# kotaro-kinoshita/yomitoku

Hardware: NVIDIA H100
Metric: pages/sec (DBNet->PARSeq OCR, synthetic 1600x1200 pages, ~200 crops/page) (higher is better)
Workload: dtype f16

## Files before the change

yomitoku_b200/csrc/gemm_tc.cu:

```cuda
#include "gemm_tc.h"

#include <cstdarg>
#include <cstdlib>
#include <cstdio>
#include <cstring>
#include <atomic>
#include <mutex>
#include <vector>

#include "ptx.cuh"

namespace ytk {

static thread_local char g_err[512] = "";
void set_error(const char* fmt, ...) {
    va_list ap;
    va_start(ap, fmt);
    vsnprintf(g_err, sizeof(g_err), fmt, ap);
    va_end(ap);
}
const char* last_error() { return g_err; }

static std::atomic<long long> g_launches{0};
void count_launch(int n) { g_launches.fetch_add(n, std::memory_order_relaxed); }
// ... 22 lines not shown
        int dev = 0;
        cudaGetDevice(&dev);
        cudaDeviceGetAttribute(&n, cudaDevAttrMultiProcessorCount, dev);
        if (n <= 0) n = 132;
    }
    return n;
}

constexpr int kBlockM = 128;
constexpr int kBlockK = 64;
constexpr int kABytes = kBlockM * kBlockK * 2;
constexpr int kThreads = 384;
constexpr int kProducerWarp = 8;
constexpr int kStagePitch = 80;
constexpr int kEpiStageBytes = 8 * 32 * kStagePitch;
constexpr int kAccPitch = 68;
constexpr int kAccBytes = 2 * 64 * kAccPitch * 4;

constexpr int kEpiBufBytes = 32 * 64;
constexpr int epi_tma_nbuf(int ) { return 2; }
constexpr int kSmemLimit = 232448;
constexpr int kSmemFixed = 1024  + 1024  + 512 ;

template <int BLOCK_N, int EPI_BYTES = kEpiStageBytes>
struct TileCfg {
    static constexpr int kBBytes = BLOCK_N * kBlockK * 2;
    static constexpr int kStageBytes = kABytes + kBBytes;
    static constexpr int kRingBudget = kSmemLimit - kSmemFixed - kAccBytes - EPI_BYTES;
    static constexpr int kStages = (kRingBudget / kStageBytes) > 8 ? 8 : (kRingBudget / kStageBytes);
    static constexpr int kRingBytes = kStages * kStageBytes;
    static constexpr int kSmemBytes = kRingBytes + kAccBytes + EPI_BYTES + kSmemFixed;
    static_assert(kStages >= 3, "K pipeline depth");
// ... 36 lines not shown
    int t2 = m_tile / a.tiles_w;
    int th = t2 % a.tiles_h;
    t.img = t2 / a.tiles_h;
    t.h0 = th * (kBlockM >> a.bw_log2);
    t.w0 = tw << a.bw_log2;
    t.n0 = n_tile * block_n;
    return t;
}

template <int BLOCK_N, int RESID, int DIRECT>
using KernelCfg = TileCfg<BLOCK_N, DIRECT == 2 ? 8 * epi_tma_nbuf(RESID) * kEpiBufBytes : kEpiStageBytes>;

template <int BLOCK_N, int OUT_F32, int RESID, int MODE, int DIRECT>
__global__ void __launch_bounds__(kThreads, 1) gemm_tc_kernel(const __grid_constant__ GemmMaps maps,
                                                              const __grid_constant__ GemmArgs args) {
    using Cfg = KernelCfg<BLOCK_N, RESID, DIRECT>;
    constexpr int kEpiBytes = Cfg::kSmemBytes - Cfg::kRingBytes - kAccBytes - kSmemFixed;
    constexpr int stage_bytes = Cfg::kStageBytes;
    constexpr int nstages = Cfg::kStages;
    extern __shared__ uint8_t smem_raw[];
    const uint32_t raw_addr = smem_u32(smem_raw);
    uint8_t* smem = smem_raw + ((1024u - (raw_addr & 1023u)) & 1023u);
    const int worker = static_cast<int>(blockIdx.x);
    const int n_workers = static_cast<int>(gridDim.x);

    float* acc_smem = reinterpret_cast<float*>(smem + Cfg::kRingBytes);
    uint8_t* epi_stage = smem + Cfg::kRingBytes + kAccBytes;
    float* fin_w = reinterpret_cast<float*>(epi_stage + kEpiBytes);
    uint64_t* full_bar = reinterpret_cast<uint64_t*>(epi_stage + kEpiBytes + 1024);
    uint64_t* empty_bar = full_bar + 8;
    [[maybe_unused]] uint64_t* rbar_base = empty_bar + 8;

    const int warp = threadIdx.x >> 5;
    const int lane = threadIdx.x & 31;

    if (threadIdx.x == 0) {
        for (int i = 0; i < nstages; ++i) {
            mbar_init(&full_bar[i], 1);
            mbar_init(&empty_bar[i], 8);
        }
        if constexpr (DIRECT == 2 && RESID != 0) {
            for (int i = 0; i < 32; ++i) mbar_init(&rbar_base[i], 1);
        }
        fence_mbar_init();
        tma_prefetch_desc(&maps.a[0]);
        tma_prefetch_desc(&maps.b);
        if constexpr (DIRECT == 2) {
            tma_prefetch_desc(&maps.out);
            if constexpr (RESID != 0) {
                tma_prefetch_desc(&maps.resid);
                tma_prefetch_desc(&maps.resid_pf);
            }
        }
    }
// ... 38 lines not shown
                    tma_load_4d(sb, &maps.b, &full_bar[stage], kb * kBlockK, tc.n0, 0, 0);
                    if (++cb == args.kpt) {
                        cb = 0;
                        ++tap;
                    }
                    if (++stage == nstages) {
                        stage = 0;
                        phase ^= 1u;
                    }
                }
            }
        }
    } else {
        setmaxnreg_inc<232>();
        const int wg = warp >> 2, wl = warp & 3;
        const int q = 2 * wg + (wl & 1);
        const int wset = wl >> 1;
        float* acc_buf = acc_smem + wg * 64 * kAccPitch;
        const float* my_acc = acc_buf + ((wl & 1) * 32 + lane) * kAccPitch;
        float acc[BLOCK_N / 2];
#pragma unroll
        for (int i = 0; i < BLOCK_N / 2; ++i) acc[i] = 0.f;
        int ring_stage = 0;
        uint32_t ring_phase = 0;
        auto mma_tile = [&]() {
            const uint32_t a_off = static_cast<uint32_t>(wg * 64 * 128);
            int prev = -1;
            for (int kb = 0; kb < num_kb; ++kb) {
                mbar_wait(&full_bar[ring_stage], ring_phase);
                const uint32_t a_addr = smem_u32(smem + ring_stage * stage_bytes);
                const uint64_t da = wgmma_desc_sw128(a_addr + a_off);
                const uint64_t db = wgmma_desc_sw128(a_addr + kABytes);
                reg_fence(acc);
                wgmma_fence();
#pragma unroll
                for (int k = 0; k < kBlockK / 16; ++k)
                    wgmma_ss<BLOCK_N>(acc, da + static_cast<uint64_t>(2 * k), db + static_cast<uint64_t>(2 * k),
                                      (kb | k) != 0 ? 1u : 0u);
                wgmma_commit();
                wgmma_wait<1>();
                reg_fence(acc);
                if (prev >= 0) {
                    __syncwarp();
                    if (lane == 0) mbar_arrive(&empty_bar[prev]);
                }
                prev = ring_stage;
                if (++ring_stage == nstages) {
                    ring_stage = 0;
                    ring_phase ^= 1u;
                }
            }
            wgmma_wait<0>();
            reg_fence(acc);
            __syncwarp();
            if (lane == 0) mbar_arrive(&empty_bar[prev]);
        };
        auto dump_slice = [&](int s) {
            named_bar_sync(1 + wg, 128);
            const int r0 = wl * 16 + (lane >> 2), c2 = (lane & 3) * 2;
#pragma unroll
            for (int j = 0; j < BLOCK_N / 8; ++j) {
                if ((j >> 3) == s) {
                    float* p = acc_buf + r0 * kAccPitch + (j & 7) * 8 + c2;
                    *reinterpret_cast<float2*>(p) = make_float2(acc[4 * j], acc[4 * j + 1]);
                    *reinterpret_cast<float2*>(p + 8 * kAccPitch) = make_float2(acc[4 * j + 2], acc[4 * j + 3]);
                }
            }
            named_bar_sync(1 + wg, 128);
        };
        auto load_chunk = [&](int c, float (&f)[32]) {
            const float4* a4 = reinterpret_cast<const float4*>(my_acc + (c & 1) * 32);
#pragma unroll
            for (int j = 0; j < 8; ++j) {
                const float4 x = a4[j];
                f[4 * j + 0] = x.x;
                f[4 * j + 1] = x.y;
                f[4 * j + 2] = x.z;
                f[4 * j + 3] = x.w;
            }
        };
        if constexpr (DIRECT == 2) {
            static_assert(MODE == EPI_NORMAL, "TMA epilogue: plain stores only");
            static_assert(RESID == 0 || (RESID == 2) == (OUT_F32 != 0), "TMA epilogue: residual and output boxes match");
            constexpr int NBUF = epi_tma_nbuf(RESID);
            constexpr int LOOK = NBUF - 1;
            constexpr int CPP = OUT_F32 ? 16 : 32;
            constexpr int NPASS = 32 / CPP;
            const int bw_mask = (1 << args.bw_log2) - 1;
            const int qw = (q * 32) & bw_mask;
            const int qh = (q * 32) >> args.bw_log2;
            uint8_t* bufs = epi_stage + warp * (NBUF * kEpiBufBytes);
            [[maybe_unused]] uint64_t* rbar = rbar_base + warp * 4;
            const int sw = args.epi_swz ? ((lane >> 1) & 3) : 0;
            const int row_off = lane * 64;
            [[maybe_unused]] int pf_u = worker, pf_c = wset, pf_p = 0, pf_g = 0;
            [[maybe_unused]] TileCoord pf_tc{};
            [[maybe_unused]] auto pf_seek = [&]() {
                while (pf_u < total_units) {
                    pf_tc = decode_tile(args, pf_u, BLOCK_N);
                    if (pf_c < BLOCK_N / 32 && pf_tc.n0 + pf_c * 32 + pf_p * CPP < args.Cout) return;
                    pf_c = wset;
                    pf_p = 0;
                    pf_u += n_workers;
                }
            };
            [[maybe_unused]] auto pf_step = [&]() {
                if (++pf_p == NPASS) {
                    pf_p = 0;
                    pf_c += 2;
                }
                pf_seek();
            };
            [[maybe_unused]] auto pf_issue = [&]() {
                const int b = pf_g % NBUF;
                mbar_expect_tx(&rbar[b], kEpiBufBytes);
                tma_load_4d(bufs + b * kEpiBufBytes, &maps.resid, &rbar[b], pf_tc.n0 + pf_c * 32 + pf_p * CPP,
                            pf_tc.w0 + qw, pf_tc.h0 + qh, pf_tc.img);
                ++pf_g;
            };
            if constexpr (RESID != 0) {
                if (lane == 0) {
                    pf_seek();
                    for (int k = 0; k < LOOK && pf_u < total_units; ++k) {
                        pf_issue();
                        pf_step();
                    }
                }
            }
            int gc = 0;
            for (int u = worker; u < total_units; u += n_workers) {
                const TileCoord tc = decode_tile(args, u, BLOCK_N);
                mma_tile();
#pragma unroll 1
                for (int c = 0; c < BLOCK_N / 32; ++c) {
                    const int col0 = tc.n0 + c * 32;
                    if ((c & 1) == 0) {
                        if (col0 >= args.Cout) break;
                        dump_slice(c >> 1);
                    }
                    if ((c & 1) != wset || col0 >= args.Cout) continue;
                    float f[32];
                    load_chunk(c, f);
                    if (args.bias != nullptr) {
                        if (col0 + 32 <= args.Cout) {
                            const float4* b4 = reinterpret_cast<const float4*>(args.bias + col0);
#pragma unroll
                            for (int j = 0; j < 8; ++j) {
                                const float4 b = __ldg(b4 + j);
                                f[4 * j + 0] += b.x;
                                f[4 * j + 1] += b.y;
                                f[4 * j + 2] += b.z;
                                f[4 * j + 3] += b.w;
                            }
                        } else {
#pragma unroll
                            for (int j = 0; j < 32; ++j) f[j] += __ldg(args.bias + min(col0 + j, args.Cout - 1));
                        }
                    }
#pragma unroll
                    for (int p = 0; p < NPASS; ++p) {
                        if (col0 + p * CPP < args.Cout) {
                            const int b = gc % NBUF;
                            uint8_t* box = bufs + b * kEpiBufBytes;
                            uint8_t* my_row = box + row_off;
                            if constexpr (RESID != 0) {
                                mbar_wait(&rbar[b], static_cast<uint32_t>(gc / NBUF) & 1u);
#pragma unroll
                                for (int j = 0; j < 4; ++j) {
                                    const uint4 r = *reinterpret_cast<const uint4*>(my_row + ((j ^ sw) << 4));
                                    if constexpr (RESID == 2) {
                                        f[p * 16 + 4 * j + 0] += __uint_as_float(r.x);
                                        f[p * 16 + 4 * j + 1] += __uint_as_float(r.y);
                                        f[p * 16 + 4 * j + 2] += __uint_as_float(r.z);
                                        f[p * 16 + 4 * j + 3] += __uint_as_float(r.w);
                                    } else {
                                        const int e = p * CPP + 8 * j;
                                        f[e + 0] += op_lo(r.x); f[e + 1] += op_hi(r.x);
                                        f[e + 2] += op_lo(r.y); f[e + 3] += op_hi(r.y);
                                        f[e + 4] += op_lo(r.z); f[e + 5] += op_hi(r.z);
                                        f[e + 6] += op_lo(r.w); f[e + 7] += op_hi(r.w);
                                    }
                                }
                            } else {
                                if (lane == 0) bulk_wait_read<NBUF - 1>();
// ... 17 lines not shown
#pragma unroll
                            for (int j = 0; j < 4; ++j) {
                                uint4 o;
                                if constexpr (OUT_F32) {
                                    o.x = __float_as_uint(f[p * 16 + 4 * j + 0]);
                                    o.y = __float_as_uint(f[p * 16 + 4 * j + 1]);
                                    o.z = __float_as_uint(f[p * 16 + 4 * j + 2]);
                                    o.w = __float_as_uint(f[p * 16 + 4 * j + 3]);
                                } else {
                                    const int e = p * CPP + 8 * j;
                                    o.x = pack_op(f[e + 0], f[e + 1]);
                                    o.y = pack_op(f[e + 2], f[e + 3]);
                                    o.z = pack_op(f[e + 4], f[e + 5]);
                                    o.w = pack_op(f[e + 6], f[e + 7]);
                                }
                                *reinterpret_cast<uint4*>(my_row + ((j ^ sw) << 4)) = o;
                            }
                            fence_proxy_async_smem();
                            __syncwarp();
                            if (lane == 0) {
                                tma_store_4d(&maps.out, box, col0 + p * CPP, tc.w0 + qw, tc.h0 + qh, tc.img);
                                bulk_commit();
                                if constexpr (RESID != 0) {
                                    if (pf_u < total_units) {
                                        bulk_wait_read<1>();
                                        pf_issue();
                                        pf_step();
                                    }
                                }
                            }
                            ++gc;
                        }
                    }
                }
            }
            if (lane == 0) bulk_wait_read<0>();
            __syncwarp();
        } else {
        constexpr bool kFin = (MODE == EPI_CONVT_FINAL);
        constexpr bool kWide = (OUT_F32 != 0) || (RESID == 2);
        constexpr int CPP = kWide ? 16 : 32;
        constexpr int NPASS = 32 / CPP;
        constexpr int OESZ = OUT_F32 ? 4 : 2;
        constexpr int RESZ = (RESID == 2) ? 4 : 2;
        const int row = q * 32 + lane;
        const int bw_mask = (1 << args.bw_log2) - 1;
        uint8_t* stage = epi_stage + warp * (32 * kStagePitch);
        uint8_t* my_row = stage + lane * kStagePitch;
        const int piece = lane & 3;
        for (int u = worker; u < total_units; u += n_workers) {
            const TileCoord tc = decode_tile(args, u, BLOCK_N);
            const int hh = tc.h0 + (row >> args.bw_log2);
            const int ww = tc.w0 + (row & bw_mask);
            const bool row_ok = (hh < args.Ho) && (ww < args.Wo);
            int c_h[4], c_w[4];
            bool c_ok[4];
#pragma unroll
            for (int it = 0; it < 4; ++it) {
                const int rr = q * 32 + it * 8 + (lane >> 2);
                c_h[it] = tc.h0 + (rr >> args.bw_log2);
                c_w[it] = tc.w0 + (rr & bw_mask);
                c_ok[it] = (c_h[it] < args.Ho) && (c_w[it] < args.Wo);
            }
            mma_tile();
            [[maybe_unused]] float dots[4] = {0.f, 0.f, 0.f, 0.f};
            [[maybe_unused]] float rm_m = -INFINITY, rm_s = 0.f;
            [[maybe_unused]] int rm_i = 0x7fffffff;
#pragma unroll 1
            for (int c = 0; c < BLOCK_N / 32; ++c) {
                const int col0 = tc.n0 + c * 32;
                if ((c & 1) == 0) {
                    if (col0 >= args.Cout) break;
                    dump_slice(c >> 1);
                }
                if (((kFin ? (c >> 1) : c) & 1) != wset) continue;
                if (col0 >= args.Cout) continue;
                [[maybe_unused]] uint4 dres[RESID == 2 ? 8 : 4];
                if constexpr (RESID != 0 && !kFin && DIRECT == 1) {
                    const long long pixo = (static_cast<long long>(tc.img) * args.Ho + hh) * args.Wo + ww;
                    const bool fullc = row_ok && (col0 + 32 <= args.Cout);
                    const uint4* gp = reinterpret_cast<const uint4*>(reinterpret_cast<const char*>(args.resid) +
                                                                     (pixo * args.ldr + col0) * RESZ);
#pragma unroll
                    for (int j = 0; j < (RESID == 2 ? 8 : 4); ++j) dres[j] = fullc ? gp[j] : make_uint4(0, 0, 0, 0);
                }
                [[maybe_unused]] uint4 rres[NPASS][4];
                if constexpr (RESID != 0 && !kFin && DIRECT == 0) {
                    constexpr int per16r = 16 / RESZ;
                    int ocol_r = col0, sub_r = 0;
                    if constexpr (MODE == EPI_SHUFFLE2X) {
                        const int cq = args.Cout >> 2;
                        sub_r = col0 / cq;
                        ocol_r = col0 - sub_r * cq;
                    }
#pragma unroll
                    for (int p = 0; p < NPASS; ++p) {
                        const int validr = min(CPP, args.Cout - (col0 + p * CPP));
                        const int e0 = piece * per16r;
#pragma unroll
                        for (int it = 0; it < 4; ++it) {
                            rres[p][it] = make_uint4(0, 0, 0, 0);
                            if (c_ok[it] && e0 + per16r <= validr) {
                                const long long pixr =
                                    (static_cast<long long>(tc.img) * args.Ho + c_h[it]) * args.Wo + c_w[it];
                                const char* gp = reinterpret_cast<const char*>(args.resid) +
                                                 (pixr * args.ldr + ocol_r + p * CPP + e0) * RESZ;
                                rres[p][it] = *reinterpret_cast<const uint4*>(gp);
                            }
                        }
                    }
                }
                float f[32];
                load_chunk(c, f);
                if (args.bias != nullptr) {
                    if (col0 + 32 <= args.Cout) {
                        const float4* b4 = reinterpret_cast<const float4*>(args.bias + col0);
#pragma unroll
                        for (int j = 0; j < 8; ++j) {
                            const float4 b = __ldg(b4 + j);
                            f[4 * j + 0] += b.x;
                            f[4 * j + 1] += b.y;
                            f[4 * j + 2] += b.z;
                            f[4 * j + 3] += b.w;
                        }
                    } else {
#pragma unroll
                        for (int j = 0; j < 32; ++j) f[j] += __ldg(args.bias + min(col0 + j, args.Cout - 1));
                    }
// ... 17 lines not shown
                        for (int j = 0; j < 32; ++j) cs += __expf(f[j] - cm);
                    }
                    if (cm > rm_m) {
                        rm_s = rm_s * __expf(rm_m - cm) + cs;
                        rm_m = cm;
                        rm_i = ci;
                    } else {
                        rm_s += cs * __expf(cm - rm_m);
                    }
                } else if constexpr (kFin) {
                    const int chan0 = (c & 1) * 32;
#pragma unroll
                    for (int j = 0; j < 32; ++j) {
                        const float x = fmaxf(f[j], 0.f);
#pragma unroll
                        for (int k = 0; k < 4; ++k) dots[k] += x * fin_w[k * 64 + chan0 + j];
                    }
                    if (c & 1) {
                        if (row_ok) {
                            const int sub = c >> 1;
                            const long long oy = 2LL * (2 * hh + (sub >> 1)), ox = 2LL * (2 * ww + (sub & 1));
                            float* op = reinterpret_cast<float*>(args.out) +
                                        (static_cast<long long>(tc.img) * (4 * args.Ho) + oy) * (4LL * args.Wo) + ox;
                            float2 r0, r1;
                            r0.x = 1.f / (1.f + __expf(-(dots[0] + args.fin_b)));
                            r0.y = 1.f / (1.f + __expf(-(dots[1] + args.fin_b)));
                            r1.x = 1.f / (1.f + __expf(-(dots[2] + args.fin_b)));
                            r1.y = 1.f / (1.f + __expf(-(dots[3] + args.fin_b)));
                            *reinterpret_cast<float2*>(op) = r0;
                            *reinterpret_cast<float2*>(op + 4LL * args.Wo) = r1;
                        }
                        dots[0] = dots[1] = dots[2] = dots[3] = 0.f;
                    }
                } else if constexpr (DIRECT == 1) {
                    int ocol = col0, sub = 0;
                    long long opix = (static_cast<long long>(tc.img) * args.Ho + hh) * args.Wo + ww;
                    if constexpr (MODE == EPI_SHUFFLE2X) {
                        const int cq = args.Cout >> 2;
                        sub = col0 / cq;
                        ocol = col0 - sub * cq;
                        opix = (static_cast<long long>(tc.img) * (2 * args.Ho) + (2 * hh + (sub >> 1))) * (2LL * args.Wo) +
                               (2 * ww + (sub & 1));
                    }
                    const bool fullc = (col0 + 32 <= args.Cout);
                    if constexpr (RESID == 2) {
                        if (fullc) {
#pragma unroll
                            for (int j = 0; j < 8; ++j) {
                                f[4 * j + 0] += __uint_as_float(dres[j].x);
                                f[4 * j + 1] += __uint_as_float(dres[j].y);
                                f[4 * j + 2] += __uint_as_float(dres[j].z);
                                f[4 * j + 3] += __uint_as_float(dres[j].w);
                            }
                        } else if (row_ok) {
                            const float* rp = reinterpret_cast<const float*>(args.resid) + opix * args.ldr + ocol;
#pragma unroll
                            for (int j = 0; j < 32; ++j)
                                if (col0 + j < args.Cout) f[j] += rp[j];
                        }
                    } else if constexpr (RESID == 1) {
                        if (fullc) {
#pragma unroll
                            for (int j = 0; j < 4; ++j) {
                                f[8 * j + 0] += op_lo(dres[j].x); f[8 * j + 1] += op_hi(dres[j].x);
                                f[8 * j + 2] += op_lo(dres[j].y); f[8 * j + 3] += op_hi(dres[j].y);
                                f[8 * j + 4] += op_lo(dres[j].z); f[8 * j + 5] += op_hi(dres[j].z);
                                f[8 * j + 6] += op_lo(dres[j].w); f[8 * j + 7] += op_hi(dres[j].w);
                            }
                        } else if (row_ok) {
                            const op_t* rp =
                                reinterpret_cast<const op_t*>(args.resid) + opix * args.ldr + ocol;
#pragma unroll
                            for (int j = 0; j < 32; ++j)
                                if (col0 + j < args.Cout) f[j] += op2f(rp[j]);
                        }
                    }
                    if (args.act == ACT_RELU) {
#pragma unroll
                        for (int j = 0; j < 32; ++j) f[j] = fmaxf(f[j], 0.f);
                    } else if (args.act == ACT_GELU) {
#pragma unroll
                        for (int j = 0; j < 32; j += 2) gelu_fast2(f[j], f[j + 1]);
                    } else if (args.act == ACT_SIGMOID) {
#pragma unroll
                        for (int j = 0; j < 32; ++j) f[j] = __fdividef(1.f, 1.f + __expf(-f[j]));
                    } else if (args.act == ACT_SILU) {
#pragma unroll
                        for (int j = 0; j < 32; ++j) f[j] = __fdividef(f[j], 1.f + __expf(-f[j]));
                    }
                    if (row_ok) {
                        if constexpr (OUT_F32) {
                            float* op = reinterpret_cast<float*>(args.out) + opix * args.ldc + ocol;
                            if (fullc) {
#pragma unroll
                                for (int j = 0; j < 8; ++j)
                                    reinterpret_cast<float4*>(op)[j] =
                                        make_float4(f[4 * j], f[4 * j + 1], f[4 * j + 2], f[4 * j + 3]);
                            } else {
#pragma unroll
                                for (int j = 0; j < 32; ++j)
                                    if (col0 + j < args.Cout) op[j] = f[j];
                            }
                        } else {
                            op_t* op = reinterpret_cast<op_t*>(args.out) + opix * args.ldc + ocol;
                            if (fullc) {
#pragma unroll
                                for (int j = 0; j < 4; ++j) {
                                    uint4 o;
                                    o.x = pack_op(f[8 * j + 0], f[8 * j + 1]);
                                    o.y = pack_op(f[8 * j + 2], f[8 * j + 3]);
                                    o.z = pack_op(f[8 * j + 4], f[8 * j + 5]);
                                    o.w = pack_op(f[8 * j + 6], f[8 * j + 7]);
                                    reinterpret_cast<uint4*>(op)[j] = o;
                                }
                            } else {
#pragma unroll
                                for (int j = 0; j < 32; ++j)
                                    if (col0 + j < args.Cout) op[j] = f2op(f[j]);
                            }
                        }
                    }
                } else {
                    int ocol = col0, sub = 0;
                    if constexpr (MODE == EPI_SHUFFLE2X) {
                        const int cq = args.Cout >> 2;
                        sub = col0 / cq;
                        ocol = col0 - sub * cq;
                    }
                    long long c_pix[4];
#pragma unroll
                    for (int it = 0; it < 4; ++it) {
                        if constexpr (MODE == EPI_SHUFFLE2X)
                            c_pix[it] = (static_cast<long long>(tc.img) * (2 * args.Ho) + (2 * c_h[it] + (sub >> 1))) *
                                            (2LL * args.Wo) +
                                        (2 * c_w[it] + (sub & 1));
                        else
                            c_pix[it] = (static_cast<long long>(tc.img) * args.Ho + c_h[it]) * args.Wo + c_w[it];
                    }
#pragma unroll
                    for (int p = 0; p < NPASS; ++p) {
                        const int pc0 = ocol + p * CPP;
                        const int valid = min(CPP, args.Cout - (col0 + p * CPP));
                        if (valid > 0) {
                            if constexpr (RESID != 0) {
                                constexpr int per16 = 16 / RESZ;
                                const int e0 = piece * per16;
#pragma unroll
                                for (int it = 0; it < 4; ++it) {
                                    const int rr = it * 8 + (lane >> 2);
                                    uint8_t* sp = stage + rr * kStagePitch + piece * 16;
                                    *reinterpret_cast<uint4*>(sp) = rres[p][it];
                                    if (c_ok[it] && e0 < valid && e0 + per16 > valid) {
                                        const char* gp = reinterpret_cast<const char*>(args.resid) +
                                                         (c_pix[it] * args.ldr + pc0 + e0) * RESZ;
                                        copy_elems(sp, gp, valid - e0, RESZ);
                                    }
                                }
                                __syncwarp();
                                if constexpr (RESID == 2) {
                                    const float4* rp = reinterpret_cast<const float4*>(my_row);
#pragma unroll
                                    for (int j = 0; j < 4; ++j) {
                                        const float4 r = rp[j];
                                        f[p * 16 + 4 * j + 0] += r.x;
                                        f[p * 16 + 4 * j + 1] += r.y;
                                        f[p * 16 + 4 * j + 2] += r.z;
                                        f[p * 16 + 4 * j + 3] += r.w;
                                    }
                                } else {
                                    const uint4* rp = reinterpret_cast<const uint4*>(my_row);
#pragma unroll
                                    for (int j = 0; j < CPP / 8; ++j) {
                                        const uint4 r = rp[j];
                                        const int b = p * CPP + 8 * j;
                                        f[b + 0] += op_lo(r.x); f[b + 1] += op_hi(r.x);
                                        f[b + 2] += op_lo(r.y); f[b + 3] += op_hi(r.y);
                                        f[b + 4] += op_lo(r.z); f[b + 5] += op_hi(r.z);
                                        f[b + 6] += op_lo(r.w); f[b + 7] += op_hi(r.w);
                                    }
                                }
                                __syncwarp();
                            }
                            if (args.act == ACT_RELU) {
#pragma unroll
                                for (int j = 0; j < CPP; ++j) f[p * CPP + j] = fmaxf(f[p * CPP + j], 0.f);
                            } else if (args.act == ACT_GELU) {
#pragma unroll
                                for (int j = 0; j < CPP; j += 2) gelu_fast2(f[p * CPP + j], f[p * CPP + j + 1]);
                            } else if (args.act == ACT_SIGMOID) {
#pragma unroll
                                for (int j = 0; j < CPP; ++j)
                                    f[p * CPP + j] = __fdividef(1.f, 1.f + __expf(-f[p * CPP + j]));
                            } else if (args.act == ACT_SILU) {
#pragma unroll
                                for (int j = 0; j < CPP; ++j)
                                    f[p * CPP + j] = __fdividef(f[p * CPP + j], 1.f + __expf(-f[p * CPP + j]));
                            }
                            if constexpr (OUT_F32) {
                                float4* wp = reinterpret_cast<float4*>(my_row);
#pragma unroll
                                for (int j = 0; j < 4; ++j) {
                                    float4 o;
                                    o.x = f[p * 16 + 4 * j + 0];
                                    o.y = f[p * 16 + 4 * j + 1];
                                    o.z = f[p * 16 + 4 * j + 2];
                                    o.w = f[p * 16 + 4 * j + 3];
                                    wp[j] = o;
                                }
                            } else {
                                uint4* wp = reinterpret_cast<uint4*>(my_row);
#pragma unroll
                                for (int j = 0; j < CPP / 8; ++j) {
                                    const int b = p * CPP + 8 * j;
                                    uint4 o;
                                    o.x = pack_op(f[b + 0], f[b + 1]);
                                    o.y = pack_op(f[b + 2], f[b + 3]);
                                    o.z = pack_op(f[b + 4], f[b + 5]);
                                    o.w = pack_op(f[b + 6], f[b + 7]);
                                    wp[j] = o;
                                }
                            }
                            __syncwarp();
                            {
                                constexpr int per16 = 16 / OESZ;
                                constexpr int row_bytes = CPP * OESZ;
// ... 15 lines not shown
                                }
                            }
                            __syncwarp();
                        }
                    }
                }
            }
            if constexpr (MODE == EPI_ROWMAX) {
                if (row_ok) {
                    const long long pixo = (static_cast<long long>(tc.img) * args.Ho + hh) * args.Wo + ww;
                    float4 o;
                    o.x = rm_m;
                    o.y = rm_s;
                    o.z = __int_as_float(rm_i);
                    o.w = 0.f;
                    reinterpret_cast<float4*>(args.out)[pixo * args.ldc + (tc.n0 / BLOCK_N) * 2 + wset] = o;
                }
            }
        }
        }
    }
}

typedef CUresult (*EncodeTiledFn)(CUtensorMap*, CUtensorMapDataType, cuuint32_t, void*, const cuuint64_t*,
                                  const cuuint64_t*, const cuuint32_t*, const cuuint32_t*, CUtensorMapInterleave,
                                  CUtensorMapSwizzle, CUtensorMapL2promotion, CUtensorMapFloatOOBfill);

static EncodeTiledFn get_encode_fn() {
    static EncodeTiledFn fn = nullptr;
    static std::once_flag once;
    std::call_once(once, []() {
// ... 62 lines not shown
                  (unsigned long long)gd[3], ld, f32, base);
        return 1;
    }
    return 0;
}

static int epi_mode_env() {
    static int mode = -1;
    if (mode < 0) {
        const char* e = getenv("YTK_EPI");
        mode = (e && e[0] == 's') ? 0 : 2;
    }
    return mode;
}

static int pick_block_n(int Cout) {
    if (Cout <= 64) return 64;
    if (Cout <= 128) return 128;
    if (Cout % 256 == 0 || Cout > 512) return 256;
    if (Cout % 128 == 0) return 128;
    return 256;
}

static int pick_bw_log2(int Ho, int Wo) {
    int best = 7;
    long long best_cost = -1;
    for (int l = 3; l <= 7; ++l) {
        int bw = 1 << l, bh = 128 >> l;
        long long cost = (long long)((Wo + bw - 1) / bw) * ((Ho + bh - 1) / bh);
        if (best_cost < 0 || cost < best_cost || (cost == best_cost && l > best)) {
            best_cost = cost;
            best = l;
        }
    }
    return best;
}

static int finish_plan(GemmPlan* plan, const void* w_packed, int Ktot, int Cout, const Epilogue& e) {
    GemmArgs& a = plan->args;
    plan->block_n = pick_block_n(Cout);
    static const bool no_shrink = getenv("YTK_NO_SHRINK") != nullptr;
    static const bool no_wave_model = getenv("YTK_WAVE_MODEL") == nullptr;
    if (e.mode != EPI_CONVT_FINAL && !no_shrink) {
        const int m_tiles = a.n_img * a.tiles_h * a.tiles_w;
        const int sms = num_sms();
        auto tiles_at = [&](int bn) { return (long long)m_tiles * ((Cout + bn - 1) / bn); };
        if (no_wave_model || (tiles_at(plan->block_n) + sms - 1) / sms > 6) {
            while (plan->block_n > 64 && tiles_at(plan->block_n) < sms) plan->block_n >>= 1;
        } else {
            int best = plan->block_n;
            double best_cost = 1e30;
            for (int bn = plan->block_n; bn >= 64; bn >>= 1) {
                const double w = bn == 256 ? 1.9 : bn == 128 ? 1.0 : 0.56;
                const double cost = (double)((tiles_at(bn) + sms - 1) / sms) * w;
                if (cost < best_cost - 1e-9) {
                    best_cost = cost;
                    best = bn;
                }
            }
            plan->block_n = best;
        }
    }
    a.tiles_n = (Cout + plan->block_n - 1) / plan->block_n;
    a.Cout = Cout;
    a.bias = e.bias;
    a.resid = e.resid;
    a.resid_f32 = e.resid_f32;
    a.ldr = e.ldr;
// ... 2 lines not shown
    a.ldc = e.ldc;
    a.act = e.act;
    a.mode = e.mode;
    a.fin_w = e.fin_w;
    a.fin_b = e.fin_b;
    if (e.out == nullptr) {
        set_error("gemm plan: null output");
        return 1;
    }
    if (e.mode == EPI_ROWMAX) {
        if (e.resid != nullptr) {
            set_error("gemm plan: ROWMAX takes no residual");
            return 1;
        }
        a.out_f32 = 1;
        a.ldc = 2LL * a.tiles_n;
    } else if (e.mode == EPI_CONVT_FINAL) {
        if (Cout != 256 || e.fin_w == nullptr || !e.out_f32) {
            set_error("gemm plan: CONVT_FINAL needs Cout=256, fp32 output and the final conv weights");
            return 1;
        }
    } else if ((e.out_f32 ? (e.ldc % 4) : (e.ldc % 8)) != 0) {
        set_error("gemm plan: ldc=%lld must keep rows 16-byte aligned", e.ldc);
        return 1;
    }
    if (e.resid && ((e.resid_f32 ? (e.ldr % 4) : (e.ldr % 8)) != 0)) {
        set_error("gemm plan: ldr=%lld must keep rows 16-byte aligned", e.ldr);
        return 1;
    }
    if (e.mode == EPI_SHUFFLE2X && ((Cout % 4) != 0 || ((Cout / 4) % 32) != 0)) {
        set_error("gemm plan: SHUFFLE2X needs Cout/4 to be a multiple of 32 (Cout=%d)", Cout);
// ... 224 lines not shown
}

template <int BLOCK_N, int OUT_F32, int RESID, int MODE>
static int launch_variant(const GemmPlan* plan, cudaStream_t stream) {
    if constexpr (MODE == EPI_NORMAL && (RESID == 0 || (RESID == 2) == (OUT_F32 != 0))) {
        if (plan->args.epi_tma) return launch_variant2<BLOCK_N, OUT_F32, RESID, MODE, 2>(plan, stream);
    }
    return launch_variant2<BLOCK_N, OUT_F32, RESID, MODE, 0>(plan, stream);
}

template <int BLOCK_N>
static int launch_bn(const GemmPlan* plan, cudaStream_t stream) {
    const GemmArgs& a = plan->args;
    const int resid = a.resid == nullptr ? 0 : (a.resid_f32 ? 2 : 1);
    if (a.mode == EPI_CONVT_FINAL) {
        if constexpr (BLOCK_N == 256) return launch_variant<256, 1, 0, EPI_CONVT_FINAL>(plan, stream);
        set_error("CONVT_FINAL needs BLOCK_N = 256");
        return 1;
    }
    if (a.mode == EPI_ROWMAX) return launch_variant2<BLOCK_N, 1, 0, EPI_ROWMAX, 0>(plan, stream);
    if (a.mode == EPI_SHUFFLE2X) {
        if (resid == 0 && !a.out_f32) return launch_variant<BLOCK_N, 0, 0, EPI_SHUFFLE2X>(plan, stream);
        if (resid == 0 && a.out_f32) return launch_variant<BLOCK_N, 1, 0, EPI_SHUFFLE2X>(plan, stream);
        set_error("SHUFFLE2X epilogue does not take a residual");
        return 1;
    }
    if (!a.out_f32) {
        if (resid == 0) return launch_variant<BLOCK_N, 0, 0, EPI_NORMAL>(plan, stream);
        if (resid == 1) return launch_variant<BLOCK_N, 0, 1, EPI_NORMAL>(plan, stream);
        return launch_variant<BLOCK_N, 0, 2, EPI_NORMAL>(plan, stream);
    }
    if (resid == 0) return launch_variant<BLOCK_N, 1, 0, EPI_NORMAL>(plan, stream);
// ... 80 lines not shown
            rec.k = g.kpt * 64;
            rec.ntaps = g.ntaps;
            rec.block_n = plan->block_n;
            rec.mode = g.mode;
            rec.act = g.act;
            rec.resid = g.resid ? (g.resid_f32 ? 2 : 1) : 0;
            rec.out_f32 = g.out_f32;
            prof = true;
        }
    }
    if (prof) cudaEventRecord(rec.a, stream);
    int rc;
    switch (plan->block_n) {
        case 64: rc = launch_bn<64>(plan, stream); break;
        case 128: rc = launch_bn<128>(plan, stream); break;
        case 256: rc = launch_bn<256>(plan, stream); break;
        default: set_error("bad block_n %d", plan->block_n); rc = 1;
    }
    if (prof) {
        cudaEventRecord(rec.b, stream);
        std::lock_guard<std::mutex> lk(g_prof_mu);
        g_prof.push_back(rec);
    }
    return rc;
}

}
```

yomitoku_b200/csrc/ptx.cuh:

```cuda
#pragma once
#include <cuda.h>
#include <cuda_bf16.h>
#include <cuda_fp16.h>
#include <cuda_runtime.h>
#include <stdint.h>
#include <string.h>

namespace ytk {

__device__ __forceinline__ uint32_t smem_u32(const void* p) {
    return static_cast<uint32_t>(__cvta_generic_to_shared(p));
}

__device__ __forceinline__ bool elect_one() {
    uint32_t pred = 0;
    asm volatile(
        "{\n\t"
        ".reg .pred P;\n\t"
        "elect.sync _|P, 0xffffffff;\n\t"
        "selp.u32 %0, 1, 0, P;\n\t"
        "}\n"
        : "=r"(pred));
    return pred != 0;
}
// ... 155 lines not shown
__device__ __forceinline__ void reg_fence(float (&d)[R]) {
#pragma unroll
    for (int i = 0; i < R; ++i) asm volatile("" : "+f"(d[i])::"memory");
}
template <int N>
__device__ __forceinline__ void setmaxnreg_dec() {
    asm volatile("setmaxnreg.dec.sync.aligned.u32 %0;" ::"n"(N));
}
template <int N>
__device__ __forceinline__ void setmaxnreg_inc() {
    asm volatile("setmaxnreg.inc.sync.aligned.u32 %0;" ::"n"(N));
}
__device__ __forceinline__ void named_bar_sync(int id, int nthreads) {
    asm volatile("bar.sync %0, %1;" ::"r"(id), "r"(nthreads) : "memory");
}

__device__ __forceinline__ uint64_t wgmma_desc_sw128(uint32_t smem_addr) {
    uint64_t d = 0;
    d |= static_cast<uint64_t>((smem_addr >> 4) & 0x3FFF);
    d |= static_cast<uint64_t>(1) << 16;
    d |= static_cast<uint64_t>(1024 >> 4) << 32;
    d |= static_cast<uint64_t>(1) << 62;
    return d;
}
__device__ __forceinline__ uint64_t wgmma_desc_sw128_mn(uint32_t smem_addr, uint32_t n_block_stride) {
    uint64_t d = 0;
    d |= static_cast<uint64_t>((smem_addr >> 4) & 0x3FFF);
    d |= static_cast<uint64_t>((n_block_stride >> 4) & 0x3FFF) << 16;
    d |= static_cast<uint64_t>(1024 >> 4) << 32;
    d |= static_cast<uint64_t>(1) << 62;
// ... 65 lines not shown
```

Baseline: 36.21.

## Ping-pong consumer warpgroups over alternating tiles so epilogue overlaps MMA

Reworks the persistent GEMM so that each of the two consumer warpgroups owns whole 128xBLOCK_N tiles on alternating units. Named barriers hand the MMA turn from one warpgroup to the other, so one group's epilogue can overlap the other's tensor-core work. The fp32 accumulator staging becomes a swizzled 32-column chunk layout, the empty barrier count drops to 4, BLOCK_N=256 is removed, and the block-size heuristics and ROWMAX/CONVT_FINAL indexing are adjusted to match. Residual loads are also software-pipelined across passes. The cost is more accumulator registers per thread (two 64-row halves), a narrower maximum N tile, and more tiles to schedule.

Result: slower. 34.65 (median of 6 runs) (-4.3%).

```diff
diff --git a/yomitoku_b200/csrc/gemm_tc.cu b/yomitoku_b200/csrc/gemm_tc.cu
--- a/yomitoku_b200/csrc/gemm_tc.cu
+++ b/yomitoku_b200/csrc/gemm_tc.cu
@@ -60,8 +60,8 @@
 constexpr int kProducerWarp = 8;
 constexpr int kStagePitch = 80;
 constexpr int kEpiStageBytes = 8 * 32 * kStagePitch;
-constexpr int kAccPitch = 68;
-constexpr int kAccBytes = 2 * 64 * kAccPitch * 4;
+constexpr int kAccBytes = 2 * kBlockM * 32 * 4;
+__device__ __forceinline__ int acc_swz(int row) { return ((row & 3) << 1) | ((row >> 2) & 1); }
 
 constexpr int kEpiBufBytes = 32 * 64;
 constexpr int epi_tma_nbuf(int ) { return 2; }
@@ -128,6 +128,8 @@
 template <int BLOCK_N, int OUT_F32, int RESID, int MODE, int DIRECT>
 __global__ void __launch_bounds__(kThreads, 1) gemm_tc_kernel(const __grid_constant__ GemmMaps maps,
                                                               const __grid_constant__ GemmArgs args) {
+    static_assert(BLOCK_N == 64 || BLOCK_N == 128, "a warpgroup owns 128 x BLOCK_N tiles, BLOCK_N <= 128");
+    static_assert(DIRECT == 0 || DIRECT == 2, "epilogue path");
     using Cfg = KernelCfg<BLOCK_N, RESID, DIRECT>;
     constexpr int kEpiBytes = Cfg::kSmemBytes - Cfg::kRingBytes - kAccBytes - kSmemFixed;
     constexpr int stage_bytes = Cfg::kStageBytes;
@@ -151,7 +153,7 @@
     if (threadIdx.x == 0) {
         for (int i = 0; i < nstages; ++i) {
             mbar_init(&full_bar[i], 1);
-            mbar_init(&empty_bar[i], 8);
+            mbar_init(&empty_bar[i], 4);
         }
         if constexpr (DIRECT == 2 && RESID != 0) {
             for (int i = 0; i < 32; ++i) mbar_init(&rbar_base[i], 1);
@@ -220,32 +222,40 @@
     } else {
         setmaxnreg_inc<232>();
         const int wg = warp >> 2, wl = warp & 3;
-        const int q = 2 * wg + (wl & 1);
-        const int wset = wl >> 1;
-        float* acc_buf = acc_smem + wg * 64 * kAccPitch;
-        const float* my_acc = acc_buf + ((wl & 1) * 32 + lane) * kAccPitch;
-        float acc[BLOCK_N / 2];
-#pragma unroll
-        for (int i = 0; i < BLOCK_N / 2; ++i) acc[i] = 0.f;
-        int ring_stage = 0;
-        uint32_t ring_phase = 0;
-        auto mma_tile = [&]() {
-            const uint32_t a_off = static_cast<uint32_t>(wg * 64 * 128);
+        float* acc_buf = acc_smem + wg * kBlockM * 32;
+        const int my_row = wl * 32 + lane;
+        const float* my_acc = acc_buf + my_row * 32;
+        const int my_swz = acc_swz(my_row);
+        float acc_lo[BLOCK_N / 2], acc_hi[BLOCK_N / 2];
+#pragma unroll
+        for (int i = 0; i < BLOCK_N / 2; ++i) acc_lo[i] = acc_hi[i] = 0.f;
+        auto mma_tile = [&](int k, bool hand_over) {
+            if (k > 0) named_bar_sync(3 + wg, 256);
+            const int pos = k * num_kb;
+            int ring_stage = pos % nstages;
+            uint32_t ring_phase = static_cast<uint32_t>(pos / nstages) & 1u;
             int prev = -1;
             for (int kb = 0; kb < num_kb; ++kb) {
                 mbar_wait(&full_bar[ring_stage], ring_phase);
                 const uint32_t a_addr = smem_u32(smem + ring_stage * stage_bytes);
-                const uint64_t da = wgmma_desc_sw128(a_addr + a_off);
+                const uint64_t da = wgmma_desc_sw128(a_addr);
+                const uint64_t da_hi = wgmma_desc_sw128(a_addr + 64 * 128);
                 const uint64_t db = wgmma_desc_sw128(a_addr + kABytes);
-                reg_fence(acc);
+                reg_fence(acc_lo);
+                reg_fence(acc_hi);
                 wgmma_fence();
 #pragma unroll
-                for (int k = 0; k < kBlockK / 16; ++k)
-                    wgmma_ss<BLOCK_N>(acc, da + static_cast<uint64_t>(2 * k), db + static_cast<uint64_t>(2 * k),
-                                      (kb | k) != 0 ? 1u : 0u);
+                for (int k16 = 0; k16 < kBlockK / 16; ++k16) {
+                    const uint32_t accum = (kb | k16) != 0 ? 1u : 0u;
+                    wgmma_ss<BLOCK_N>(acc_lo, da + static_cast<uint64_t>(2 * k16), db + static_cast<uint64_t>(2 * k16),
+                                      accum);
+                    wgmma_ss<BLOCK_N>(acc_hi, da_hi + static_cast<uint64_t>(2 * k16),
+                                      db + static_cast<uint64_t>(2 * k16), accum);
+                }
                 wgmma_commit();
                 wgmma_wait<1>();
-                reg_fence(acc);
+                reg_fence(acc_lo);
+                reg_fence(acc_hi);
                 if (prev >= 0) {
                     __syncwarp();
                     if (lane == 0) mbar_arrive(&empty_bar[prev]);
@@ -256,29 +266,34 @@
                     ring_phase ^= 1u;
                 }
             }
+            if (hand_over) named_bar_arrive(3 + (wg ^ 1), 256);
             wgmma_wait<0>();
-            reg_fence(acc);
+            reg_fence(acc_lo);
+            reg_fence(acc_hi);
             __syncwarp();
             if (lane == 0) mbar_arrive(&empty_bar[prev]);
         };
-        auto dump_slice = [&](int s) {
+        auto dump_chunk = [&](int c) {
             named_bar_sync(1 + wg, 128);
             const int r0 = wl * 16 + (lane >> 2), c2 = (lane & 3) * 2;
+            const int swz = acc_swz(r0);
 #pragma unroll
             for (int j = 0; j < BLOCK_N / 8; ++j) {
-                if ((j >> 3) == s) {
-                    float* p = acc_buf + r0 * kAccPitch + (j & 7) * 8 + c2;
-                    *reinterpret_cast<float2*>(p) = make_float2(acc[4 * j], acc[4 * j + 1]);
-                    *reinterpret_cast<float2*>(p + 8 * kAccPitch) = make_float2(acc[4 * j + 2], acc[4 * j + 3]);
+                if ((j >> 2) == c) {
+                    float* p = acc_buf + r0 * 32 + ((((j & 3) * 2 + (c2 >> 2)) ^ swz) << 2) + (c2 & 3);
+                    *reinterpret_cast<float2*>(p) = make_float2(acc_lo[4 * j], acc_lo[4 * j + 1]);
+                    *reinterpret_cast<float2*>(p + 8 * 32) = make_float2(acc_lo[4 * j + 2], acc_lo[4 * j + 3]);
+                    *reinterpret_cast<float2*>(p + 64 * 32) = make_float2(acc_hi[4 * j], acc_hi[4 * j + 1]);
+                    *reinterpret_cast<float2*>(p + 72 * 32) = make_float2(acc_hi[4 * j + 2], acc_hi[4 * j + 3]);
                 }
             }
             named_bar_sync(1 + wg, 128);
         };
-        auto load_chunk = [&](int c, float (&f)[32]) {
-            const float4* a4 = reinterpret_cast<const float4*>(my_acc + (c & 1) * 32);
+        auto load_chunk = [&](float (&f)[32]) {
+            const float4* a4 = reinterpret_cast<const float4*>(my_acc);
 #pragma unroll
             for (int j = 0; j < 8; ++j) {
-                const float4 x = a4[j];
+                const float4 x = a4[j ^ my_swz];
                 f[4 * j + 0] = x.x;
                 f[4 * j + 1] = x.y;
                 f[4 * j + 2] = x.z;
@@ -293,27 +308,27 @@
             constexpr int CPP = OUT_F32 ? 16 : 32;
             constexpr int NPASS = 32 / CPP;
             const int bw_mask = (1 << args.bw_log2) - 1;
-            const int qw = (q * 32) & bw_mask;
-            const int qh = (q * 32) >> args.bw_log2;
+            const int qw = (wl * 32) & bw_mask;
+            const int qh = (wl * 32) >> args.bw_log2;
             uint8_t* bufs = epi_stage + warp * (NBUF * kEpiBufBytes);
             [[maybe_unused]] uint64_t* rbar = rbar_base + warp * 4;
             const int sw = args.epi_swz ? ((lane >> 1) & 3) : 0;
             const int row_off = lane * 64;
-            [[maybe_unused]] int pf_u = worker, pf_c = wset, pf_p = 0, pf_g = 0;
+            [[maybe_unused]] int pf_u = worker + wg * n_workers, pf_c = 0, pf_p = 0, pf_g = 0;
             [[maybe_unused]] TileCoord pf_tc{};
             [[maybe_unused]] auto pf_seek = [&]() {
                 while (pf_u < total_units) {
                     pf_tc = decode_tile(args, pf_u, BLOCK_N);
                     if (pf_c < BLOCK_N / 32 && pf_tc.n0 + pf_c * 32 + pf_p * CPP < args.Cout) return;
-                    pf_c = wset;
+                    pf_c = 0;
                     pf_p = 0;
-                    pf_u += n_workers;
+                    pf_u += 2 * n_workers;
                 }
             };
             [[maybe_unused]] auto pf_step = [&]() {
                 if (++pf_p == NPASS) {
                     pf_p = 0;
-                    pf_c += 2;
+                    ++pf_c;
                 }
                 pf_seek();
             };
@@ -334,19 +349,16 @@
                 }
             }
             int gc = 0;
-            for (int u = worker; u < total_units; u += n_workers) {
+            for (int u = worker + wg * n_workers, k = wg; u < total_units; u += 2 * n_workers, k += 2) {
                 const TileCoord tc = decode_tile(args, u, BLOCK_N);
-                mma_tile();
+                mma_tile(k, u + n_workers < total_units);
 #pragma unroll 1
                 for (int c = 0; c < BLOCK_N / 32; ++c) {
                     const int col0 = tc.n0 + c * 32;
-                    if ((c & 1) == 0) {
-                        if (col0 >= args.Cout) break;
-                        dump_slice(c >> 1);
-                    }
-                    if ((c & 1) != wset || col0 >= args.Cout) continue;
+                    if (col0 >= args.Cout) break;
+                    dump_chunk(c);
                     float f[32];
-                    load_chunk(c, f);
+                    load_chunk(f);
                     if (args.bias != nullptr) {
                         if (col0 + 32 <= args.Cout) {
                             const float4* b4 = reinterpret_cast<const float4*>(args.bias + col0);
@@ -368,12 +380,12 @@
                         if (col0 + p * CPP < args.Cout) {
                             const int b = gc % NBUF;
                             uint8_t* box = bufs + b * kEpiBufBytes;
-                            uint8_t* my_row = box + row_off;
+                            uint8_t* my_box_row = box + row_off;
                             if constexpr (RESID != 0) {
                                 mbar_wait(&rbar[b], static_cast<uint32_t>(gc / NBUF) & 1u);
 #pragma unroll
                                 for (int j = 0; j < 4; ++j) {
-                                    const uint4 r = *reinterpret_cast<const uint4*>(my_row + ((j ^ sw) << 4));
+                                    const uint4 r = *reinterpret_cast<const uint4*>(my_box_row + ((j ^ sw) << 4));
                                     if constexpr (RESID == 2) {
                                         f[p * 16 + 4 * j + 0] += __uint_as_float(r.x);
                                         f[p * 16 + 4 * j + 1] += __uint_as_float(r.y);
@@ -421,7 +433,7 @@
                                     o.z = pack_op(f[e + 4], f[e + 5]);
                                     o.w = pack_op(f[e + 6], f[e + 7]);
                                 }
-                                *reinterpret_cast<uint4*>(my_row + ((j ^ sw) << 4)) = o;
+                                *reinterpret_cast<uint4*>(my_box_row + ((j ^ sw) << 4)) = o;
                             }
                             fence_proxy_async_smem();
                             __syncwarp();
@@ -450,75 +462,53 @@
         constexpr int NPASS = 32 / CPP;
         constexpr int OESZ = OUT_F32 ? 4 : 2;
         constexpr int RESZ = (RESID == 2) ? 4 : 2;
-        const int row = q * 32 + lane;
         const int bw_mask = (1 << args.bw_log2) - 1;
         uint8_t* stage = epi_stage + warp * (32 * kStagePitch);
-        uint8_t* my_row = stage + lane * kStagePitch;
+        uint8_t* my_stage_row = stage + lane * kStagePitch;
         const int piece = lane & 3;
-        for (int u = worker; u < total_units; u += n_workers) {
+        for (int u = worker + wg * n_workers, k = wg; u < total_units; u += 2 * n_workers, k += 2) {
             const TileCoord tc = decode_tile(args, u, BLOCK_N);
-            const int hh = tc.h0 + (row >> args.bw_log2);
-            const int ww = tc.w0 + (row & bw_mask);
+            const int hh = tc.h0 + (my_row >> args.bw_log2);
+            const int ww = tc.w0 + (my_row & bw_mask);
             const bool row_ok = (hh < args.Ho) && (ww < args.Wo);
             int c_h[4], c_w[4];
             bool c_ok[4];
 #pragma unroll
             for (int it = 0; it < 4; ++it) {
-                const int rr = q * 32 + it * 8 + (lane >> 2);
+                const int rr = wl * 32 + it * 8 + (lane >> 2);
                 c_h[it] = tc.h0 + (rr >> args.bw_log2);
                 c_w[it] = tc.w0 + (rr & bw_mask);
                 c_ok[it] = (c_h[it] < args.Ho) && (c_w[it] < args.Wo);
             }
-            mma_tile();
+            mma_tile(k, u + n_workers < total_units);
             [[maybe_unused]] float dots[4] = {0.f, 0.f, 0.f, 0.f};
             [[maybe_unused]] float rm_m = -INFINITY, rm_s = 0.f;
             [[maybe_unused]] int rm_i = 0x7fffffff;
 #pragma unroll 1
             for (int c = 0; c < BLOCK_N / 32; ++c) {
                 const int col0 = tc.n0 + c * 32;
-                if ((c & 1) == 0) {
-                    if (col0 >= args.Cout) break;
-                    dump_slice(c >> 1);
-                }
-                if (((kFin ? (c >> 1) : c) & 1) != wset) continue;
-                if (col0 >= args.Cout) continue;
-                [[maybe_unused]] uint4 dres[RESID == 2 ? 8 : 4];
-                if constexpr (RESID != 0 && !kFin && DIRECT == 1) {
-                    const long long pixo = (static_cast<long long>(tc.img) * args.Ho + hh) * args.Wo + ww;
-                    const bool fullc = row_ok && (col0 + 32 <= args.Cout);
-                    const uint4* gp = reinterpret_cast<const uint4*>(reinterpret_cast<const char*>(args.resid) +
-                                                                     (pixo * args.ldr + col0) * RESZ);
-#pragma unroll
-                    for (int j = 0; j < (RESID == 2 ? 8 : 4); ++j) dres[j] = fullc ? gp[j] : make_uint4(0, 0, 0, 0);
-                }
-                [[maybe_unused]] uint4 rres[NPASS][4];
-                if constexpr (RESID != 0 && !kFin && DIRECT == 0) {
+                if (col0 >= args.Cout) break;
+                [[maybe_unused]] uint4 rres[4];
+                [[maybe_unused]] auto load_resid = [&](int p) {
                     constexpr int per16r = 16 / RESZ;
-                    int ocol_r = col0, sub_r = 0;
-                    if constexpr (MODE == EPI_SHUFFLE2X) {
-                        const int cq = args.Cout >> 2;
-                        sub_r = col0 / cq;
-                        ocol_r = col0 - sub_r * cq;
-                    }
-#pragma unroll
-                    for (int p = 0; p < NPASS; ++p) {
-                        const int validr = min(CPP, args.Cout - (col0 + p * CPP));
-                        const int e0 = piece * per16r;
-#pragma unroll
-                        for (int it = 0; it < 4; ++it) {
-                            rres[p][it] = make_uint4(0, 0, 0, 0);
-                            if (c_ok[it] && e0 + per16r <= validr) {
-                                const long long pixr =
-                                    (static_cast<long long>(tc.img) * args.Ho + c_h[it]) * args.Wo + c_w[it];
-                                const char* gp = reinterpret_cast<const char*>(args.resid) +
-                                                 (pixr * args.ldr + ocol_r + p * CPP + e0) * RESZ;
-                                rres[p][it] = *reinterpret_cast<const uint4*>(gp);
-                            }
+                    const int validr = min(CPP, args.Cout - (col0 + p * CPP));
+                    const int e0 = piece * per16r;
+#pragma unroll
+                    for (int it = 0; it < 4; ++it) {
+                        rres[it] = make_uint4(0, 0, 0, 0);
+                        if (c_ok[it] && e0 + per16r <= validr) {
+                            const long long pixr =
+                                (static_cast<long long>(tc.img) * args.Ho + c_h[it]) * args.Wo + c_w[it];
+                            const char* gp = reinterpret_cast<const char*>(args.resid) +
+                                             (pixr * args.ldr + col0 + p * CPP + e0) * RESZ;
+                            rres[it] = *reinterpret_cast<const uint4*>(gp);
                         }
                     }
-                }
+                };
+                if constexpr (RESID != 0 && !kFin) load_resid(0);
+                dump_chunk(c);
                 float f[32];
-                load_chunk(c, f);
+                load_chunk(f);
                 if (args.bias != nullptr) {
                     if (col0 + 32 <= args.Cout) {
                         const float4* b4 = reinterpret_cast<const float4*>(args.bias + col0);
@@ -566,11 +556,11 @@
                     for (int j = 0; j < 32; ++j) {
                         const float x = fmaxf(f[j], 0.f);
 #pragma unroll
-                        for (int k = 0; k < 4; ++k) dots[k] += x * fin_w[k * 64 + chan0 + j];
+                        for (int kk = 0; kk < 4; ++kk) dots[kk] += x * fin_w[kk * 64 + chan0 + j];
                     }
                     if (c & 1) {
                         if (row_ok) {
-                            const int sub = c >> 1;
+                            const int sub = (tc.n0 >> 6) + (c >> 1);
                             const long long oy = 2LL * (2 * hh + (sub >> 1)), ox = 2LL * (2 * ww + (sub & 1));
                             float* op = reinterpret_cast<float*>(args.out) +
                                         (static_cast<long long>(tc.img) * (4 * args.Ho) + oy) * (4LL * args.Wo) + ox;
@@ -584,94 +574,6 @@
                         }
                         dots[0] = dots[1] = dots[2] = dots[3] = 0.f;
                     }
-                } else if constexpr (DIRECT == 1) {
-                    int ocol = col0, sub = 0;
-                    long long opix = (static_cast<long long>(tc.img) * args.Ho + hh) * args.Wo + ww;
-                    if constexpr (MODE == EPI_SHUFFLE2X) {
-                        const int cq = args.Cout >> 2;
-                        sub = col0 / cq;
-                        ocol = col0 - sub * cq;
-                        opix = (static_cast<long long>(tc.img) * (2 * args.Ho) + (2 * hh + (sub >> 1))) * (2LL * args.Wo) +
-                               (2 * ww + (sub & 1));
-                    }
-                    const bool fullc = (col0 + 32 <= args.Cout);
-                    if constexpr (RESID == 2) {
-                        if (fullc) {
-#pragma unroll
-                            for (int j = 0; j < 8; ++j) {
-                                f[4 * j + 0] += __uint_as_float(dres[j].x);
-                                f[4 * j + 1] += __uint_as_float(dres[j].y);
-                                f[4 * j + 2] += __uint_as_float(dres[j].z);
-                                f[4 * j + 3] += __uint_as_float(dres[j].w);
-                            }
-                        } else if (row_ok) {
-                            const float* rp = reinterpret_cast<const float*>(args.resid) + opix * args.ldr + ocol;
-#pragma unroll
-                            for (int j = 0; j < 32; ++j)
-                                if (col0 + j < args.Cout) f[j] += rp[j];
-                        }
-                    } else if constexpr (RESID == 1) {
-                        if (fullc) {
-#pragma unroll
-                            for (int j = 0; j < 4; ++j) {
-                                f[8 * j + 0] += op_lo(dres[j].x); f[8 * j + 1] += op_hi(dres[j].x);
-                                f[8 * j + 2] += op_lo(dres[j].y); f[8 * j + 3] += op_hi(dres[j].y);
-                                f[8 * j + 4] += op_lo(dres[j].z); f[8 * j + 5] += op_hi(dres[j].z);
-                                f[8 * j + 6] += op_lo(dres[j].w); f[8 * j + 7] += op_hi(dres[j].w);
-                            }
-                        } else if (row_ok) {
-                            const op_t* rp =
-                                reinterpret_cast<const op_t*>(args.resid) + opix * args.ldr + ocol;
-#pragma unroll
-                            for (int j = 0; j < 32; ++j)
-                                if (col0 + j < args.Cout) f[j] += op2f(rp[j]);
-                        }
-                    }
-                    if (args.act == ACT_RELU) {
-#pragma unroll
-                        for (int j = 0; j < 32; ++j) f[j] = fmaxf(f[j], 0.f);
-                    } else if (args.act == ACT_GELU) {
-#pragma unroll
-                        for (int j = 0; j < 32; j += 2) gelu_fast2(f[j], f[j + 1]);
-                    } else if (args.act == ACT_SIGMOID) {
-#pragma unroll
-                        for (int j = 0; j < 32; ++j) f[j] = __fdividef(1.f, 1.f + __expf(-f[j]));
-                    } else if (args.act == ACT_SILU) {
-#pragma unroll
-                        for (int j = 0; j < 32; ++j) f[j] = __fdividef(f[j], 1.f + __expf(-f[j]));
-                    }
-                    if (row_ok) {
-                        if constexpr (OUT_F32) {
-                            float* op = reinterpret_cast<float*>(args.out) + opix * args.ldc + ocol;
-                            if (fullc) {
-#pragma unroll
-                                for (int j = 0; j < 8; ++j)
-                                    reinterpret_cast<float4*>(op)[j] =
-                                        make_float4(f[4 * j], f[4 * j + 1], f[4 * j + 2], f[4 * j + 3]);
-                            } else {
-#pragma unroll
-                                for (int j = 0; j < 32; ++j)
-                                    if (col0 + j < args.Cout) op[j] = f[j];
-                            }
-                        } else {
-                            op_t* op = reinterpret_cast<op_t*>(args.out) + opix * args.ldc + ocol;
-                            if (fullc) {
-#pragma unroll
-                                for (int j = 0; j < 4; ++j) {
-                                    uint4 o;
-                                    o.x = pack_op(f[8 * j + 0], f[8 * j + 1]);
-                                    o.y = pack_op(f[8 * j + 2], f[8 * j + 3]);
-                                    o.z = pack_op(f[8 * j + 4], f[8 * j + 5]);
-                                    o.w = pack_op(f[8 * j + 6], f[8 * j + 7]);
-                                    reinterpret_cast<uint4*>(op)[j] = o;
-                                }
-                            } else {
-#pragma unroll
-                                for (int j = 0; j < 32; ++j)
-                                    if (col0 + j < args.Cout) op[j] = f2op(f[j]);
-                            }
-                        }
-                    }
                 } else {
                     int ocol = col0, sub = 0;
                     if constexpr (MODE == EPI_SHUFFLE2X) {
@@ -701,7 +603,7 @@
                                 for (int it = 0; it < 4; ++it) {
                                     const int rr = it * 8 + (lane >> 2);
                                     uint8_t* sp = stage + rr * kStagePitch + piece * 16;
-                                    *reinterpret_cast<uint4*>(sp) = rres[p][it];
+                                    *reinterpret_cast<uint4*>(sp) = rres[it];
                                     if (c_ok[it] && e0 < valid && e0 + per16 > valid) {
                                         const char* gp = reinterpret_cast<const char*>(args.resid) +
                                                          (c_pix[it] * args.ldr + pc0 + e0) * RESZ;
@@ -709,8 +611,9 @@
                                     }
                                 }
                                 __syncwarp();
+                                if (p + 1 < NPASS) load_resid(p + 1);
                                 if constexpr (RESID == 2) {
-                                    const float4* rp = reinterpret_cast<const float4*>(my_row);
+                                    const float4* rp = reinterpret_cast<const float4*>(my_stage_row);
 #pragma unroll
                                     for (int j = 0; j < 4; ++j) {
                                         const float4 r = rp[j];
@@ -720,7 +623,7 @@
                                         f[p * 16 + 4 * j + 3] += r.w;
                                     }
                                 } else {
-                                    const uint4* rp = reinterpret_cast<const uint4*>(my_row);
+                                    const uint4* rp = reinterpret_cast<const uint4*>(my_stage_row);
 #pragma unroll
                                     for (int j = 0; j < CPP / 8; ++j) {
                                         const uint4 r = rp[j];
@@ -749,7 +652,7 @@
                                     f[p * CPP + j] = __fdividef(f[p * CPP + j], 1.f + __expf(-f[p * CPP + j]));
                             }
                             if constexpr (OUT_F32) {
-                                float4* wp = reinterpret_cast<float4*>(my_row);
+                                float4* wp = reinterpret_cast<float4*>(my_stage_row);
 #pragma unroll
                                 for (int j = 0; j < 4; ++j) {
                                     float4 o;
@@ -760,7 +663,7 @@
                                     wp[j] = o;
                                 }
                             } else {
-                                uint4* wp = reinterpret_cast<uint4*>(my_row);
+                                uint4* wp = reinterpret_cast<uint4*>(my_stage_row);
 #pragma unroll
                                 for (int j = 0; j < CPP / 8; ++j) {
                                     const int b = p * CPP + 8 * j;
@@ -806,7 +709,7 @@
                     o.y = rm_s;
                     o.z = __int_as_float(rm_i);
                     o.w = 0.f;
-                    reinterpret_cast<float4*>(args.out)[pixo * args.ldc + (tc.n0 / BLOCK_N) * 2 + wset] = o;
+                    reinterpret_cast<float4*>(args.out)[pixo * args.ldc + tc.n0 / BLOCK_N] = o;
                 }
             }
         }
@@ -899,13 +802,7 @@
     return mode;
 }
 
-static int pick_block_n(int Cout) {
-    if (Cout <= 64) return 64;
-    if (Cout <= 128) return 128;
-    if (Cout % 256 == 0 || Cout > 512) return 256;
-    if (Cout % 128 == 0) return 128;
-    return 256;
-}
+static int pick_block_n(int Cout) { return Cout <= 64 ? 64 : 128; }
 
 static int pick_bw_log2(int Ho, int Wo) {
     int best = 7;
@@ -931,12 +828,12 @@
         const int sms = num_sms();
         auto tiles_at = [&](int bn) { return (long long)m_tiles * ((Cout + bn - 1) / bn); };
         if (no_wave_model || (tiles_at(plan->block_n) + sms - 1) / sms > 6) {
-            while (plan->block_n > 64 && tiles_at(plan->block_n) < sms) plan->block_n >>= 1;
+            while (plan->block_n > 64 && tiles_at(plan->block_n) < 2 * sms) plan->block_n >>= 1;
         } else {
             int best = plan->block_n;
             double best_cost = 1e30;
             for (int bn = plan->block_n; bn >= 64; bn >>= 1) {
-                const double w = bn == 256 ? 1.9 : bn == 128 ? 1.0 : 0.56;
+                const double w = bn == 128 ? 1.0 : 0.56;
                 const double cost = (double)((tiles_at(bn) + sms - 1) / sms) * w;
                 if (cost < best_cost - 1e-9) {
                     best_cost = cost;
@@ -969,7 +866,7 @@
             return 1;
         }
         a.out_f32 = 1;
-        a.ldc = 2LL * a.tiles_n;
+        a.ldc = a.tiles_n;
     } else if (e.mode == EPI_CONVT_FINAL) {
         if (Cout != 256 || e.fin_w == nullptr || !e.out_f32) {
             set_error("gemm plan: CONVT_FINAL needs Cout=256, fp32 output and the final conv weights");
@@ -1224,8 +1121,8 @@
     const GemmArgs& a = plan->args;
     const int resid = a.resid == nullptr ? 0 : (a.resid_f32 ? 2 : 1);
     if (a.mode == EPI_CONVT_FINAL) {
-        if constexpr (BLOCK_N == 256) return launch_variant<256, 1, 0, EPI_CONVT_FINAL>(plan, stream);
-        set_error("CONVT_FINAL needs BLOCK_N = 256");
+        if constexpr (BLOCK_N == 128) return launch_variant<128, 1, 0, EPI_CONVT_FINAL>(plan, stream);
+        set_error("CONVT_FINAL needs BLOCK_N = 128");
         return 1;
     }
     if (a.mode == EPI_ROWMAX) return launch_variant2<BLOCK_N, 1, 0, EPI_ROWMAX, 0>(plan, stream);
@@ -1336,7 +1233,6 @@
     switch (plan->block_n) {
         case 64: rc = launch_bn<64>(plan, stream); break;
         case 128: rc = launch_bn<128>(plan, stream); break;
-        case 256: rc = launch_bn<256>(plan, stream); break;
         default: set_error("bad block_n %d", plan->block_n); rc = 1;
     }
     if (prof) {
diff --git a/yomitoku_b200/csrc/ptx.cuh b/yomitoku_b200/csrc/ptx.cuh
--- a/yomitoku_b200/csrc/ptx.cuh
+++ b/yomitoku_b200/csrc/ptx.cuh
@@ -193,6 +193,9 @@
 __device__ __forceinline__ void named_bar_sync(int id, int nthreads) {
     asm volatile("bar.sync %0, %1;" ::"r"(id), "r"(nthreads) : "memory");
 }
+__device__ __forceinline__ void named_bar_arrive(int id, int nthreads) {
+    asm volatile("bar.arrive %0, %1;" ::"r"(id), "r"(nthreads) : "memory");
+}
 
 __device__ __forceinline__ uint64_t wgmma_desc_sw128(uint32_t smem_addr) {
     uint64_t d = 0;
```
